# benabbouosama/DEEPL-Project

Measured on AMD Instinct MI355X. Metric: images/sec train step, TransVAE-Large f16d32 256px bs256, higher is better.
Workload: dtype bf16

## Files before the change

### deepl-project_amd/csrc/igemm_common.h

```cpp
#pragma once
#pragma clang fp contract(off)
#include "common.h"

#include <type_traits>

namespace tvi {

struct IgemmArgs {
    const bf16* x;
    const bf16* w;
    const float* bias;
    const bf16* res;
    const bf16* aux;
    bf16* pre;
    bf16* out;
    const char* zeros;
    int M, N, K;
    int batch, h_in, w_in, c_in, ldx;
    int h_out, w_out, ldo;
    int kh, kw, stride, pad, up_shift, dil_mask;
    int tiles_n, tiles_m, xcd_order;
    int sup_r, sup_c;
    int tpb, nchunks;
    int shuffle;
    int act;
    int aux_act;
    int pre_deriv;
    int form;
    const float* rope;
    int rope_tokens, rope_cols;
    int hw_shift, w_shift;
    unsigned dv_hw_m, dv_w_m, dv_cq_m;
    int dv_hw_s, dv_w_s, dv_cq_s;
    int store_nt;
    unsigned out_bytes;
    unsigned x_bytes, w_bytes;
    const bf16* x2;
    unsigned x2_bytes;
    int ldx2, k1_steps;
};

constexpr int LDS_MAX = 160 * 1024;
extern int g_cfg_bm, g_cfg_bn, g_halo_ring;
extern bool g_halo_w4, g_xcd_order, g_epi_modes;
int epilogue_mode(const IgemmArgs& a);
int pick_tile(long long M, int N, bool allow256, bool allow192_256rows, int* bm);
int launch_halo(IgemmArgs& a, hipStream_t s);
#ifdef TV_PROBE
int set_halo_probe(void* dev_buf);
#endif

}

namespace {
using namespace tvi;

#ifndef TV_NO_PIPE2
#define TV_NO_PIPE2 0
#endif
#ifndef TV_NO_LOADER_SPLIT
#define TV_NO_LOADER_SPLIT 1
#endif
#ifndef TV_HALO_VOFF_REGS
#define TV_HALO_VOFF_REGS 1
#endif
#ifndef TV_HALO_BURST
#define TV_HALO_BURST 1
#endif
#ifndef TV_GENERIC_BURST
#define TV_GENERIC_BURST 1
#endif
#ifndef TV_PIPE_ALL_MAX
// ... 672 lines not shown
```

### deepl-project_amd/csrc/igemm_nt.hip

```cpp
#include "igemm_common.h"

namespace tvi {
int g_cfg_bm = 0;
int g_cfg_bn = 0;
int g_halo_ring = 3;
bool g_halo_w4 = false;
bool g_xcd_order = true;
int g_supertile = 0;
bool g_epi_modes = true;

int epilogue_mode(const IgemmArgs& a) {
    if (a.rope) return 0;
    if (!g_epi_modes || a.shuffle || a.pre || a.out_bytes == 0) return 0;
    if (a.aux) return (a.aux_act == TV_ACT_DERIV && !a.res) ? 2 : 0;
    return (a.res && a.act == TV_ACT_NONE) ? 1 : 0;
}

int pick_tile(long long M, int N, bool allow256, bool allow192_256rows, int* bm) {
    const long long m256 = (M + 255) / 256, m128 = (M + 127) / 128;
    double best = 1e30;
    int bn = 128;
    *bm = 128;
    auto consider = [&](int cbn, int cbm, long long tiles, double slots, double eff) {
        const double rounds = (double)((long long)((tiles + slots - 1) / slots));
// ... 112 lines not shown
            } else {
                b = m / hw;
                const int r = m - b * hw;
                oy = r / p.w_out;
                ox = r - oy * p.w_out;
            }
            a_oy[it] = oy * p.stride - p.pad;
            a_ox[it] = ox * p.stride - p.pad;
            a_pix[it] = b * p.h_in * p.w_in;
        } else {
            a_oy[it] = -(1 << 28);
            a_ox[it] = 0;
            a_pix[it] = 0;
        }
    }
    const bf16* b_src[B_IT];
    bool b_ok[B_IT];
    int b_voff[B_IT];
#pragma unroll
    for (int it = 0; it < B_IT; ++it) {
        const int j = it * NW + wave;
        const int row = j * RPI + srow;
        const int rl = row % WTN;
        const int fi = bfrag_reader(rl);
        const int c = (sslot ^ swz_of<BK>(fi)) * 8;
        const int n = n0 + row;
        b_ok[it] = (j < B_INSTR) && (n < p.N);
        b_src[it] = p.w + (size_t)(b_ok[it] ? n : 0) * p.K + c;
        b_voff[it] = b_ok[it] ? (n * p.K + c) * 2 : OOB_OFFSET;
    }

    const int cch = p.c_in / BK;
#ifdef TV_ABL_K1
    const int nk = 1;
#else
    const int nk = p.kh * p.kw * cch;
#endif
    int st_ky = 0, st_kx = 0, st_ch = 0, st_t = 0;
    [[maybe_unused]] int st_i = walk_i, st_am = m0 * p.ldx * 2, st_nb = n0 * p.K * 2;
    const bf16* a_src[A_IT];
    bool a_ok[A_IT];
    int a_voff[A_IT];
    const int hv = p.h_in << p.up_shift, wv = p.w_in << p.up_shift;

    auto tap_setup = [&]() {
#pragma unroll
        for (int it = 0; it < A_IT; ++it) {
            const int uy = a_oy[it] + st_ky, ux = a_ox[it] + st_kx;
            const bool ok = ((unsigned)uy < (unsigned)hv) && ((unsigned)ux < (unsigned)wv) &&
                            (((uy | ux) & p.dil_mask) == 0);
            const int iy = uy >> p.up_shift, ix = ux >> p.up_shift;
            const int pix = a_pix[it] + iy * p.w_in + ix;
            a_ok[it] = ok;
            if constexpr (BUF) a_voff[it] = ok ? (pix * p.ldx + a_chunk[it]) * 2 : OOB_OFFSET;
            else a_src[it] = p.x + (size_t)(ok ? pix : 0) * p.ldx + a_chunk[it];
        }
    };
    tap_setup();

    bf16x8 a_reg[DMA ? 1 : A_IT], b_reg[DMA ? 1 : B_IT];

    auto issue_piece = [&](char* sbase, int q) {
        if (q < A_IT) {
            const int it = q, j = it * NW + wave;
            const int koff = st_ch * BK;
            if (A_INSTR % NW != 0 && j >= A_INSTR) {
                if constexpr (PADDED && BUF) buffer_load_lds16(p.x, p.x_bytes, smem + STAGES * STAGE, OOB_OFFSET, 0);
                else if constexpr (PADDED) __builtin_amdgcn_global_load_lds(TV_GLB(p.zeros + lane * 16), TV_LDS(smem + STAGES * STAGE), 16, 0, 0);
                return;
            }
            if constexpr (BUF) {
                buffer_load_lds16(p.x, p.x_bytes, sbase + j * 1024, a_voff[it], koff * 2 + (PERSIST ? st_am : 0));
            } else if constexpr (DMA) {
                const void* src = a_ok[it] ? (const void*)(a_src[it] + koff) : (const void*)(p.zeros + lane * 16);
                __builtin_amdgcn_global_load_lds(TV_GLB(src), TV_LDS(sbase + j * 1024), 16, 0, 0);
            } else {
// ... 7 lines not shown
            if (B_INSTR % NW != 0 && j >= B_INSTR) {
                if constexpr (PADDED && BUF) buffer_load_lds16(p.w, p.w_bytes, smem + STAGES * STAGE, OOB_OFFSET, 0);
                else if constexpr (PADDED) __builtin_amdgcn_global_load_lds(TV_GLB(p.zeros + lane * 16), TV_LDS(smem + STAGES * STAGE), 16, 0, 0);
                return;
            }
            if constexpr (BUF) {
                buffer_load_lds16(p.w, p.w_bytes, sbase + A_BYTES + j * 1024, b_voff[it], kb * 2 + (PERSIST ? st_nb : 0));
            } else if constexpr (DMA) {
                const void* src = b_ok[it] ? (const void*)(b_src[it] + kb) : (const void*)(p.zeros + lane * 16);
                __builtin_amdgcn_global_load_lds(TV_GLB(src), TV_LDS(sbase + A_BYTES + j * 1024), 16, 0, 0);
            } else {
                bf16x8 v = {0, 0, 0, 0, 0, 0, 0, 0};
                if (b_ok[it]) v = *(const bf16x8*)(b_src[it] + kb);
                b_reg[it] = v;
            }
        }
    };
    auto stage_advance = [&]() {
        if constexpr (PERSIST) {
            ++st_t;
            ++st_ch;
            if (st_t == nk) {
                st_i += p.nchunks;
                const int r = st_i / p.tiles_n, c = st_i - r * p.tiles_n;
                st_am = (r * 8 + walk_x) * (BM * p.ldx * 2);
                st_nb = c * (BN * p.K * 2);
                st_t = st_ch = 0;
            }
            return;
        }
        ++st_t;
        if (++st_ch == cch) {
            st_ch = 0;
            if (++st_kx == p.kw) {
                st_kx = 0;
                ++st_ky;
            }
            if (st_t < nk) tap_setup();
        }
    };
    auto stage_issue = [&](char* sbase) {
#pragma unroll
        for (int q = 0; q < NI; ++q) issue_piece(sbase, q);
        stage_advance();
    };
    auto stage_write = [&](char* sbase) {
        if constexpr (!DMA) {
#pragma unroll
            for (int it = 0; it < A_IT; ++it) {
                const int j = it * NW + wave;
                if (A_INSTR % NW != 0 && j >= A_INSTR) break;
                *(bf16x8*)(sbase + j * 1024 + lane * 16) = a_reg[it];
            }
#pragma unroll
            for (int it = 0; it < B_IT; ++it) {
                const int j = it * NW + wave;
                if (B_INSTR % NW != 0 && j >= B_INSTR) break;
                *(bf16x8*)(sbase + A_BYTES + j * 1024 + lane * 16) = b_reg[it];
            }
        }
    };

    int fi = lane & 15, fq = lane >> 4;
    int sw = swz_of<BK>(fi);
    int a_row_off = (wm * WTM + fi) * (BK * 2);
    int b_row_off = A_BYTES + (wn * WTN + bfrag_lane_row(fi)) * (BK * 2);
    [[maybe_unused]] auto persist_reinit = [&]() {
        int tl = threadIdx.x;
        asm volatile("" : "+v"(tl));
        const int ln = tl & 63, sr = ln / CPR, ss = ln % CPR;
#pragma unroll
// ... 466 lines not shown
            compute(smem + (t & 1) * STAGE, nullptr, std::false_type{});
            if (t + 1 < nk) stage_write(smem + ((t + 1) & 1) * STAGE);
        }
    }

    if (TV_SETPRIO) __builtin_amdgcn_s_setprio(0);
    TV_T(5);
#ifdef TV_ABL_NO_EPI
    {
        float chk = 0.f;
#pragma unroll
        for (int i = 0; i < MF; ++i)
#pragma unroll
            for (int j = 0; j < NF; ++j) chk += acc[i][j][0] + acc[i][j][1] + acc[i][j][2] + acc[i][j][3];
        if (chk != 123.456f) return;
    }
#endif
    f32x4 bvals[NF];
    load_bias<WTN>(p, lane, n0 + wn * WTN, bvals);
    const int mrow0 = m0 + wm * WTM;
    epilogue<WTM, WTN, EPI, MODE == 2 && (BM * BN >= 128 * 128)>(p, acc, bvals, smem, wave, lane, n0 + wn * WTN, [&](int r) { return mrow0 + r; });
    TV_T(6);
    TV_PROBE_DUMP(wave, lane);
}

bool g_use_dma = true;
int g_nt_threshold_mb = 64;
int g_loop8 = 1;
int g_persist = 0;
int g_cfg_stages = 0;
int g_cfg_bk = 0;
int g_addr_mode = 0;
bool g_use_halo = true;





int epilogue_form(const IgemmArgs& a) {
    if (!g_epi_modes) return EF_GENERIC;
    if (a.shuffle) {
        if (a.rope || ((a.N >> 2) % 64) != 0 || (a.N & 3)) return EF_GENERIC;
        if (a.shuffle == 1) {
            if (a.aux) return (a.aux_act == TV_ACT_DERIV && !a.res && !a.pre && a.act == TV_ACT_NONE) ? EF_DERIV_S1 : EF_GENERIC;
            if (a.pre || a.act != TV_ACT_NONE) return EF_GENERIC;
            return a.res ? EF_RES_S1 : EF_PLAIN_S1;
        }
        if (a.aux || a.res) return EF_GENERIC;
        if (a.pre) return (a.pre_deriv && a.act == TV_ACT_SILU) ? EF_SILU_D_S2 : EF_GENERIC;
        return a.act == TV_ACT_NONE ? EF_PLAIN_S2 : EF_GENERIC;
    }
    if (a.rope) return (!a.aux && !a.res && !a.pre && a.act == TV_ACT_NONE && a.rope_cols % 32 == 0) ? EF_ROPE : EF_GENERIC;
    if (a.aux) {
        if (a.aux_act == TV_ACTX_RELU) return (!a.res && !a.pre && a.act == TV_ACT_NONE) ? EF_RELU_MASK : EF_GENERIC;
        if (a.aux_act == TV_ACTX_LRELU) return (!a.res && !a.pre && a.act == TV_ACT_NONE) ? EF_LRELU_MASK : EF_GENERIC;
        if (!a.res || a.pre || a.act != TV_ACT_NONE) return EF_GENERIC;
        return a.aux_act == TV_ACT_DERIV ? EF_RES_DERIV : (a.aux_act == TV_ACT_ADD ? EF_RES2 : EF_GENERIC);
    }
    if (a.res) return EF_GENERIC;
    if (a.pre) {
        if (!a.pre_deriv) return EF_GENERIC;
        return a.act == TV_ACT_GELU ? EF_GELU_D : (a.act == TV_ACT_SILU ? EF_SILU_D : EF_GENERIC);
    }
    if (a.act == TV_ACTX_RELU) return EF_RELU;
    if (a.act == TV_ACTX_LRELU) return EF_LRELU;
    return a.act == TV_ACT_NONE ? EF_PLAIN : (a.act == TV_ACT_GELU ? EF_GELU : (a.act == TV_ACT_SILU ? EF_SILU : EF_GENERIC));
// ... 92 lines not shown
                    hipLaunchKernelGGL((igemm_nt_kernel<BM, BN, WGM, WGN, BK, STAGES, MODE, EPI_MODE, false, 0, true>), grid, block, BYTES, s, a);
                    return;
                }
            }
            hipLaunchKernelGGL((igemm_nt_kernel<BM, BN, WGM, WGN, BK, STAGES, MODE, EPI_MODE>), grid, block, BYTES, s, a);
        };
        const int epi = epilogue_mode(a);
        if constexpr (MODE == 2 && BM * BN >= 128 * 128) {
            if (epi == 1) { go(std::integral_constant<int, 1>{}); return 0; }
            if (epi == 2) { go(std::integral_constant<int, 2>{}); return 0; }
        }
        go(std::integral_constant<int, 0>{});
        return 0;
    }
}

template <int BN, int BK, int MODE>
int launch_big(const IgemmArgs& a, int bm, int stages, hipStream_t s) {
    constexpr int WGM8 = (BN == 256) ? 2 : 4, WGN8 = (BN == 256) ? 4 : 2;
    if constexpr (MODE == 0) {
        return launch_one<128, BN, 2, 2, BK, 2, 0>(a, s);
    } else {
        if (bm == 256) {
            if (stages >= 3 && launch_one<256, BN, WGM8, WGN8, BK, 3, MODE>(a, s) == 0) return 0;
            return launch_one<256, BN, WGM8, WGN8, BK, 2, MODE>(a, s);
        }
        if (stages >= 3 && launch_one<128, BN, 2, 2, BK, 3, MODE>(a, s) == 0) return 0;
        return launch_one<128, BN, 2, 2, BK, 2, MODE>(a, s);
    }
}



template <int BK, int MODE>
int launch_mode(IgemmArgs& a, hipStream_t s) {
    const int N = a.N;
    const int stages = g_cfg_stages ? g_cfg_stages : 2;
    if (N > 64) {
        int bm = 128;
        int bn = pick_tile(a.M, N, true, true, &bm);
        if (g_cfg_bn == 256 && N % 256 == 0) { bn = 256; bm = 256; }
        else if (g_cfg_bn == 192 && N % 192 == 0) { bn = 192; bm = 256; }
        else if (g_cfg_bn == 128) { bn = (N % 192 == 0 && N % 128 != 0) ? 192 : 128; bm = 128; }
        if (g_cfg_bm) bm = g_cfg_bm;
        if (bn == 256) {
            a.tiles_n = N / 256;
            return launch_big<256, BK, MODE>(a, bm, stages, s);
        }
        if (bn == 192) {
            a.tiles_n = N / 192;
            return launch_big<192, BK, MODE>(a, bm, stages, s);
        }
        a.tiles_n = (N + 127) / 128;
        return launch_big<128, BK, MODE>(a, bm, stages, s);
    }
    a.tiles_n = 1;
    if (N > 32) return launch_one<128, 64, 2, 2, BK, 2, MODE>(a, s);
    return launch_one<128, 32, 4, 1, BK, 2, MODE>(a, s);
}

template <int BK>
int launch_bk(IgemmArgs& a, hipStream_t s) {
    if (!g_use_dma) return launch_mode<BK, 0>(a, s);
    if (g_addr_mode != 1 && a.x_bytes != 0 && a.w_bytes != 0) return launch_mode<BK, 2>(a, s);
    return launch_mode<BK, 1>(a, s);
}

}

extern "C" int tv_set_dma(int on) {
    g_use_dma = on != 0;
    g_addr_mode = (on == 2) ? 1 : 0;
    return 0;
}

extern "C" int tv_set_igemm_halo(int on) {
    g_halo_w4 = on >= 100;
    on %= 100;
    g_xcd_order = on < 10;
    on %= 10;
    g_use_halo = on != 0;
    g_halo_ring = (on == 2) ? 2 : (on == 4 ? 4 : 3);
    return 0;
}

extern "C" int tv_set_igemm_nt_threshold(int mib) {
    g_nt_threshold_mb = mib;
    return 0;
}

extern "C" int tv_set_igemm_persist(int on) {
    if (on == -1) g_loop8 = 0;
    else if (on == -2) g_loop8 = 1;
    else g_persist = on;
    return 0;
}

extern "C" int tv_set_igemm_supertile(int v) {
    g_supertile = v;
    return 0;
}

extern "C" int tv_set_igemm_epilogue(int on) {
    g_epi_modes = on != 0;
    return 0;
}

#ifdef TV_PROBE
extern "C" int tv_set_igemm_probe(void* dev_buf) {
    const bool ok = hipMemcpyToSymbol(HIP_SYMBOL(g_probe_dev), &dev_buf, sizeof(void*)) == hipSuccess;
    return (tvi::set_halo_probe(dev_buf) == 0 && ok) ? 0 : 1;
}
#endif

extern "C" int tv_set_igemm_config(int bm, int bn, int stages, int bk) {
    g_cfg_bm = bm;
// ... 27 lines not shown
extern "C" int tv_igemm_nt(const tv_conv_desc* d, const void* x, const void* w, const float* bias,
                           const void* residual, void* pre_act, void* out, void* stream) {
    return igemm_nt_impl(d, x, w, bias, residual, pre_act, out, nullptr, TV_ACT_NONE, stream);
}

extern "C" int tv_igemm_nt_actgrad(const tv_conv_desc* d, const void* x, const void* w, const void* residual,
                                   const void* aux_pre_act, int aux_act, void* out, void* stream) {
    TV_CHECK_ARG(aux_pre_act && aux_act >= 0 && aux_act <= TV_ACTX_LRELU && d && d->act == TV_ACT_NONE,
                 "tv_igemm_nt_actgrad: needs the saved pre-activation, a valid activation id and desc.act == NONE");
    return igemm_nt_impl(d, x, w, nullptr, residual, nullptr, out, aux_pre_act, aux_act, stream);
}

extern "C" int tv_igemm_nt_cat2(const tv_conv_desc* d, const void* x, const void* x2, int k1, int ldx2, const void* w, const float* bias,
                               const void* residual, const void* aux, int aux_act, void* out, void* stream) {
    TV_CHECK_ARG(x2 && d && d->act == TV_ACT_NONE && (!aux || (aux_act >= 0 && aux_act <= TV_ACT_ADD && !bias)),
                 "tv_igemm_nt_cat2: needs the second source, desc.act == NONE, and no bias together with aux");
    return igemm_nt_impl(d, x, w, bias, residual, nullptr, out, aux, aux ? aux_act : TV_ACT_NONE, stream, RopeSpec{nullptr, 0, 0}, Cat2Spec{x2, k1, ldx2});
}

static int igemm_nt_impl(const tv_conv_desc* d, const void* x, const void* w, const float* bias, const void* residual,
                         void* pre_act, void* out, const void* aux, int aux_act, void* stream, RopeSpec rope, Cat2Spec cat) {
    TV_CHECK_ARG(d && x && w && out, "tv_igemm_nt: null pointer");
    if (cat.x2) {
        TV_CHECK_ARG(d->kh == 1 && d->kw == 1 && d->stride == 1 && d->pad == 0 && d->up_shift == 0 && d->dil_mask == 0 && d->store_shuffle == 0 && !rope.tab,
                     "tv_igemm_nt_cat2: single-tap layers only");
        TV_CHECK_ARG(cat.k1 > 0 && cat.k1 % 64 == 0 && d->c_in > cat.k1 && (d->c_in - cat.k1) % 64 == 0 && d->ldx >= cat.k1 && d->ldx % 8 == 0 &&
                     cat.ldx2 >= d->c_in - cat.k1 && cat.ldx2 % 8 == 0, "tv_igemm_nt_cat2: k1=%d c_in=%d ldx=%d ldx2=%d", cat.k1, d->c_in, d->ldx, cat.ldx2);
    }
    TV_CHECK_ARG(d->c_in > 0 && d->c_in % 32 == 0, "tv_igemm_nt: c_in=%d must be a multiple of 32", d->c_in);
    TV_CHECK_ARG(d->c_out > 0 && d->c_out % 8 == 0, "tv_igemm_nt: c_out=%d must be a multiple of 8", d->c_out);
    TV_CHECK_ARG(cat.x2 || (d->ldx >= d->c_in && d->ldx % 8 == 0), "tv_igemm_nt: ldx=%d (c_in=%d) must be >= c_in and a multiple of 8", d->ldx, d->c_in);
    TV_CHECK_ARG(d->ldo % 8 == 0, "tv_igemm_nt: ldo=%d must be a multiple of 8", d->ldo);
    TV_CHECK_ARG(d->batch > 0 && d->h_in > 0 && d->w_in > 0 && d->h_out > 0 && d->w_out > 0, "tv_igemm_nt: empty geometry");
    TV_CHECK_ARG(d->kh > 0 && d->kw > 0 && d->stride > 0 && d->pad >= 0, "tv_igemm_nt: bad taps");
    TV_CHECK_ARG((d->up_shift | 1) == 1 && (d->dil_mask | 1) == 1, "tv_igemm_nt: up_shift/dil_mask must be 0 or 1");
    TV_CHECK_ARG(d->act >= 0 && ((d->act & ~TV_ACT_SAVE_DERIV) <= 2 || d->act == TV_ACTX_RELU || d->act == TV_ACTX_LRELU), "tv_igemm_nt: unknown activation %d", d->act);
    TV_CHECK_ARG(!(d->act & TV_ACT_SAVE_DERIV) || (pre_act && (d->act & ~TV_ACT_SAVE_DERIV) != TV_ACT_NONE),
                 "tv_igemm_nt: TV_ACT_SAVE_DERIV needs an activation and a pre_act buffer");
    TV_CHECK_ARG((d->act != TV_ACTX_RELU && d->act != TV_ACTX_LRELU) || !pre_act, "tv_igemm_nt: a ReLU / LeakyReLU layer saves nothing (its output is its own backward mask): pre_act must be NULL");
    TV_CHECK_ARG(d->store_shuffle >= 0 && d->store_shuffle <= 2, "tv_igemm_nt: store_shuffle must be 0, 1 or 2");
    const long long M = (long long)d->batch * d->h_out * d->w_out;
    TV_CHECK_ARG(M < (1ll << 31) && (long long)d->batch * d->h_in * d->w_in < (1ll << 31), "tv_igemm_nt: too many pixels");
    if (d->store_shuffle) {
        TV_CHECK_ARG(d->c_out % 32 == 0 && d->ldo >= d->c_out / 4, "tv_igemm_nt: shuffle store needs c_out %% 32 == 0");
    } else {
        TV_CHECK_ARG(d->ldo >= d->c_out, "tv_igemm_nt: ldo < c_out");
    }
    if (tv_init() != TV_OK) return TV_ERR_INIT;

    IgemmArgs a;
    a.x = (const bf16*)x;
    a.w = (const bf16*)w;
    a.bias = bias;
    a.res = (const bf16*)residual;
    a.aux = (const bf16*)aux;
    a.aux_act = aux_act;
    a.pre = (bf16*)pre_act;
    a.out = (bf16*)out;
    a.zeros = (const char*)tv_zero_page();
    a.M = (int)M;
    a.N = d->c_out;
    a.K = d->kh * d->kw * d->c_in;
    a.batch = d->batch; a.h_in = d->h_in; a.w_in = d->w_in; a.c_in = d->c_in; a.ldx = d->ldx;
    a.h_out = d->h_out; a.w_out = d->w_out; a.ldo = d->ldo;
    a.kh = d->kh; a.kw = d->kw; a.stride = d->stride; a.pad = d->pad;
    a.up_shift = d->up_shift; a.dil_mask = d->dil_mask;
    a.tiles_n = 1;
    a.shuffle = d->store_shuffle;
    a.act = d->act & ~TV_ACT_SAVE_DERIV;
    a.pre_deriv = (d->act & TV_ACT_SAVE_DERIV) ? 1 : 0;
    a.rope = rope.tab;
    a.rope_tokens = rope.tokens;
    a.rope_cols = rope.cols;
    a.form = epilogue_form(a);
    {
        auto lg = [](int v) { int s = 0; while ((1 << s) < v) ++s; return ((1 << s) == v) ? s : -1; };
        a.w_shift = lg(d->w_out);
        a.hw_shift = lg(d->h_out * d->w_out);
        if (a.hw_shift < 0 || a.w_shift < 0) a.hw_shift = a.w_shift = -1;
    }
    {
        auto fd = [](int d, unsigned& m, int& sh) {
            if (d <= 1) { m = 0; sh = 0; return; }
            int L = 0;
            while ((1ll << L) < d) ++L;
            m = (unsigned)(((1ull << (31 + L)) + (unsigned long long)d - 1) / (unsigned long long)d);
            sh = L - 1;
        };
        fd(d->h_out * d->w_out, a.dv_hw_m, a.dv_hw_s);
        fd(d->w_out, a.dv_w_m, a.dv_w_s);
        fd(a.N >> 2, a.dv_cq_m, a.dv_cq_s);
    }
    {
        const long long rows = (long long)d->batch * d->h_in * d->w_in;
        const long long xb = (rows - 1) * d->ldx * 2 + (long long)(cat.x2 ? cat.k1 : d->c_in) * 2;
        const long long wb = (long long)a.N * a.K * 2;
        a.x_bytes = xb < (1ll << 31) ? (unsigned)xb : 0u;
        a.w_bytes = wb < (1ll << 31) ? (unsigned)wb : 0u;
        a.x2 = (const bf16*)cat.x2;
        a.ldx2 = cat.x2 ? cat.ldx2 : d->ldx;
// ... 25 lines not shown
```

### deepl-project_amd/transvae/hip/_lib.py

```python
from __future__ import annotations

import ctypes as C
import glob
import os
import subprocess
import threading

_HERE = os.path.dirname(os.path.abspath(__file__))
PKG_ROOT = os.path.dirname(os.path.dirname(_HERE))
CSRC = os.path.join(PKG_ROOT, "csrc")
SO_PATH = os.environ.get("TV_HIP_SO") or os.path.join(_HERE, "libtransvae_hip.so")

ACT_NONE, ACT_GELU, ACT_SILU = 0, 1, 2
ACT_DERIV, ACT_SAVE_DERIV = 3, 16
ACT_ADD = 4
ACTX_RELU = 5
ACTX_LRELU = 6
GAN_GEN, GAN_BCE, GAN_HINGE, GAN_WGAN = 0, 1, 2, 3
LPIPS_MAP, LPIPS_SIGMOID, LPIPS_CLAMP = 1, 2, 4
POOL3_MAX_S2, POOL3_MAX_S1P1, POOL3_AVG_S1P1 = 0, 1, 2
SSIM_SKIMAGE, SSIM_BOX11 = 0, 1
METRIC_NONE, METRIC_CLIP, METRIC_SIGMOID = 0, 1, 2
IMAGE_NONE, IMAGE_SIGMOID = 0, 1
ERR_UNSUPPORTED = 4
DERIVE_UP_FWD, DERIVE_UP_DGRAD, DERIVE_UP_WGRAD_FOLD, DERIVE_S2_PARITY = 1, 2, 3, 4


class ConvDesc(C.Structure):
    _fields_ = [(n, C.c_int) for n in (
        "batch", "h_in", "w_in", "c_in", "ldx",
        "h_out", "w_out", "c_out", "ldo",
        "kh", "kw", "stride", "pad",
        "up_shift", "dil_mask", "act", "store_shuffle")]


class ImageDesc(C.Structure):
    _fields_ = [("offset", C.c_longlong)] + [(n, C.c_int) for n in (
        "in_h", "in_w", "row_stride", "channels", "out_h", "out_w", "crop_top", "crop_left", "xtab", "xk", "ytab", "yk")]


_P, _I, _F, _LL = C.c_void_p, C.c_int, C.c_float, C.c_longlong
_DP = C.POINTER(ConvDesc)

SIGNATURES = {
    "tv_init": (_I, []),
    "tv_last_error": (C.c_char_p, []),
    "tv_abi_version": (_I, []),
    "tv_igemm_nt": (_I, [_DP, _P, _P, _P, _P, _P, _P, _P]),
    "tv_igemm_nt_rope": (_I, [_DP, _P, _P, _P, _P, _P, _I, _I, _P]),
    "tv_igemm_nt_actgrad": (_I, [_DP, _P, _P, _P, _P, _I, _P, _P]),
    "tv_igemm_nt_cat2": (_I, [_DP, _P, _P, _I, _I, _P, _P, _P, _P, _I, _P, _P]),
    "tv_wgrad_tn": (_I, [_DP, _P, _P, _P, _P, _P]),
    "tv_wgrad_tn_overwrites": (_I, [_DP]),
    "tv_wgrad_tn_acc": (_I, [_DP, _P, _P, _P, _P, _P]),
    "tv_pack_weight": (_I, [_P, _P, _P, _I, _I, _I, _I, _P]),
    "tv_conv3x3_derived": (_I, [_P, _P, _I, _I, _I, _I, _P]),
    "tv_gn_partial_count": (_LL, [_I, _I, _I]),
    "tv_gn_stats": (_I, [_P, _P, _P, _I, _I, _I, _P]),
    "tv_gn_silu_fwd": (_I, [_P, _P, _P, _P, _P, _P, _I, _I, _I, _I, _F, _P]),
    "tv_gn_silu_apply": (_I, [_P, _P, _P, _P, _P, _I, _I, _I, _I, _P]),
    "tv_gn_silu_bwd_reduce": (_I, [_P, _P, _P, _P, _P, _P, _P, _I, _I, _I, _I, _P]),
    "tv_gn_silu_bwd_apply": (_I, [_P, _P, _P, _P, _P, _P, _P, _P, _P, _P, _I, _I, _I, _I, _P]),
    "tv_rownorm_fwd": (_I, [_P, _P, _P, _I, _I, _I, _F, _F, _P]),
    "tv_rownorm_bwd": (_I, [_P, _P, _P, _P, _P, _P, _I, _I, _I, _F, _F, _P]),
    "tv_rope_qk": (_I, [_P, _P, _I, _I, _I, _I, _P]),
    "tv_attn_fwd": (_I, [_P, _P, _P, _I, _I, _I, _F, _P]),
    "tv_attn_bwd": (_I, [_P, _P, _P, _P, _P, _P, _P, _I, _I, _I, _F, _P]),
    "tv_act_bwd": (_I, [_P, _P, _P, _LL, _I, _P]),
    "tv_add_": (_I, [_P, _P, _LL, _P]),
    "tv_nchw_to_nhwc": (_I, [_P, _P, _I, _I, _I, _I, _I, _P]),
    "tv_nhwc_to_nchw": (_I, [_P, _P, _I, _I, _I, _I, _I, _P]),
    "tv_im2col3x3": (_I, [_P, _P, _I, _I, _I, _I, _I, _P]),
    "tv_pool2x2_sum": (_I, [_P, _P, _I, _I, _I, _I, _P]),
    "tv_fold_cols": (_I, [_P, _P, _P, _P, _P, _I, _I, _P]),
    "tv_fold_partial_count": (_LL, [_I, _I]),
    "tv_fold_cols_bwd": (_I, [_P, _P, _P, _P, _P, _P, _P, _P, _P, _I, _I, _P]),
    "tv_vae_loss_partial_count": (_LL, [_LL, _LL]),
    "tv_vae_loss_l1_kl": (_I, [_P, _P, _P, _P, _P, _P, _P, _P, _P, _LL, _LL, _F, _F, _F, _I, _F, _F, _P]),
    "tv_opt_chunk_elems": (_I, []),
    "tv_opt_grad_norm": (_I, [_P, _P, _I, _P, _P, _F, _F, _F, _I, _P]),
    "tv_opt_adamw": (_I, [_P, _P, _I, _P, _F, _F, _F, _F, _F, _P]),
# ... 140 lines not shown
```

### deepl-project_amd/transvae/hip/ops.py

```python
from __future__ import annotations

import contextlib
import ctypes as C
import functools
from typing import Optional

import torch

from . import _lib as L

BF16 = torch.bfloat16


def _p(t: Optional[torch.Tensor]):
    return None if t is None else C.c_void_p(t.data_ptr())


def _stream():
    return C.c_void_p(torch.cuda.current_stream().cuda_stream)


def _require(cond: bool, msg: str):
    if not cond:
        raise RuntimeError("transvae.hip: " + msg)
# ... 113 lines not shown
                        L.check(L.load().tv_pack_weight(_p(w), None, _p(dt), O, T, I, int(flip), _stream()), "tv_pack_weight")
                        ent.forms[fk] = dt
                return d, dt
    key = None
    if _pack_cache is not None and is_param:
        key = (id(base), base._version, w.data_ptr(), O, T, I, want_fwd, want_t, flip)
        hit = _pack_cache.get(key)
        if hit is not None:
            return hit
    d = torch.empty((O, T, I), dtype=BF16, device=w.device) if want_fwd else None
    dt = torch.empty((I, T, O), dtype=BF16, device=w.device) if want_t else None
    lib = L.load()
    L.check(lib.tv_pack_weight(_p(w), _p(d), _p(dt), O, T, I, int(flip), _stream()), "tv_pack_weight")
    if key is not None:
        _pack_cache[key] = (d, dt)
    return d, dt


def _derived_weight(w: torch.Tensor, kind: str, build):
    if _pack_cache is None:
        return build()
    base = w._base if w._base is not None else w
    if not isinstance(base, torch.nn.Parameter):
        return build()
    key = (id(base), base._version, w.data_ptr(), tuple(w.shape), kind)
    hit = _pack_cache.get(key)
    if hit is None:
        hit = _pack_cache[key] = build()
    return hit


def _desc(**kw) -> L.ConvDesc:
    d = L.ConvDesc()
    for k in ("up_shift", "dil_mask", "act", "store_shuffle", "pad"):
        setattr(d, k, 0)
    d.stride = 1
    for k, v in kw.items():
        setattr(d, k, int(v))
    return d


_LAUNCH_BYTES = (1 << 31) - (1 << 26)


def _batch_chunks(batch: int, tensors, align: int = 1):
    per_row = 0
    for t in tensors:
        if t is not None:
            per_row = max(per_row, (t.numel() // batch) * t.element_size())
    if per_row * batch < _LAUNCH_BYTES:
        return None
    rows = max(align, (_LAUNCH_BYTES // per_row) // align * align)
    n = -(-batch // rows)
    rows = -(-(-(-batch // n)) // align) * align
    return [(s, min(rows, batch - s)) for s in range(0, batch, rows)]


def _row_ptr(t, batch: int, row: int):
    if t is None:
        return None
    return C.c_void_p(t.data_ptr() + row * (t.numel() // batch) * t.element_size())


def _desc_rows(desc: L.ConvDesc, rows: int) -> L.ConvDesc:
    d = L.ConvDesc()
    C.memmove(C.byref(d), C.byref(desc), C.sizeof(L.ConvDesc))
    d.batch = rows
# ... 245 lines not shown
        lib = L.load()
        B = desc.batch
        for s, c in (_batch_chunks(B, (gz, residual, aux, dx)) or [(0, B)]):
            L.check(lib.tv_igemm_nt_actgrad(C.byref(_desc_rows(desc, c)), _row_ptr(gz, B, s), _p(wt), _row_ptr(residual, B, s),
                                            _row_ptr(aux, B, s), aux_act, _row_ptr(dx, B, s), _stream()), "tv_igemm_nt_actgrad")


_UP_SETS = (((0,), (1, 2)), ((0, 1), (2,)))


def _derive(w: torch.Tensor, form: int, Cout: int, Cin: int, out: torch.Tensor, accumulate: bool = False) -> torch.Tensor:
    _require(w.dtype == torch.float32 and w.is_contiguous() and out.is_contiguous(), "derived operand needs contiguous fp32 input")
    L.check(L.load().tv_conv3x3_derived(_p(w), _p(out), form, Cout, Cin, int(accumulate), _stream()), "tv_conv3x3_derived")
    return out


def _up_fwd_weight(w: torch.Tensor, Cout: int, Cin: int) -> torch.Tensor:
    return _derive(w.view(Cout, 3, 3, Cin), L.DERIVE_UP_FWD, Cout, Cin, torch.empty((4 * Cout, 2, 2, Cin), dtype=BF16, device=w.device))


_UP_ADJ = ((2,), (1, 2), (0, 1), (0,))


def _up_dgrad_weight(w: torch.Tensor, Cout: int, Cin: int) -> torch.Tensor:
    return _derive(w.view(Cout, 3, 3, Cin), L.DERIVE_UP_DGRAD, Cout, Cin, torch.empty((Cin, 4, 4, Cout), dtype=BF16, device=w.device))


def _up_fold_wgrad(d16: torch.Tensor, Cout: int, Cin: int, out: Optional[torch.Tensor] = None, accumulate: bool = False) -> torch.Tensor:
    if out is None:
        out = torch.empty((Cout, 3, 3, Cin), dtype=torch.float32, device=d16.device)
    return _derive(d16, L.DERIVE_UP_WGRAD_FOLD, Cout, Cin, out, accumulate)


def _s2_parity_weight(w: torch.Tensor, Cout: int, Cin: int) -> torch.Tensor:
    return _derive(w.view(Cout, 3, 3, Cin), L.DERIVE_S2_PARITY, Cout, Cin, torch.empty((4 * Cin, 2, 2, Cout), dtype=BF16, device=w.device))


def _rows_desc(rows: int, c_in: int, c_out: int) -> L.ConvDesc:
    return _desc(batch=rows, h_in=1, w_in=1, c_in=c_in, ldx=c_in, h_out=1, w_out=1, c_out=c_out, ldo=c_out, kh=1, kw=1)


def gemm_rows(x: torch.Tensor, wb: torch.Tensor, c_out: int, bias=None, residual=None, aux=None, aux_act: int = 0) -> torch.Tensor:
    T, K = x.shape
    out = torch.empty((T, c_out), dtype=BF16, device=x.device)
    d = _rows_desc(T, K, c_out)
    if aux is None:
        igemm(d, x, wb, bias, residual, None, out)
    else:
        _require(bias is None, "gemm_rows: bias and a derivative multiply do not combine")
        _igemm_bwd(d, x, wb, residual, aux, aux_act, out)
    return out


def gemm_rows2(x1: torch.Tensor, x2: torch.Tensor, wb: torch.Tensor, c_out: int, bias=None, residual=None, aux=None, aux_act: int = 0):
    T, K1 = x1.shape
    K2 = x2.shape[1]
    _require(x1.dtype == BF16 and x2.dtype == BF16 and x1.is_contiguous() and x2.is_contiguous() and x2.shape[0] == T and
             wb.dtype == BF16 and wb.is_contiguous() and
             (tuple(wb.shape[-2:]) == (c_out, K1 + K2) or wb.numel() == c_out * (K1 + K2)), "gemm_rows2: operand check failed")
    if K1 % 64 or K2 % 64 or _batch_chunks(T, (x1, x2, residual, aux)) is not None:
        return None
    d = _rows_desc(T, K1 + K2, c_out)
    d.ldx = K1
    out = torch.empty((T, c_out), dtype=BF16, device=x1.device)
    rc = L.load().tv_igemm_nt_cat2(C.byref(d), _p(x1), _p(x2), K1, K2, _p(wb), _p(bias), _p(residual), _p(aux), int(aux_act), _p(out), _stream())
    if rc == 4:
# ... 129 lines not shown


def _c4s2_poly_weight(w: torch.Tensor, Cout: int, Cin: int) -> torch.Tensor:
    wt = w.permute(3, 1, 2, 0)
    out = torch.empty((4, Cin, 2, 2, Cout), dtype=BF16, device=w.device)
    for py in range(2):
        for px in range(2):
            sel = wt[:, list(_C4S2_KY[py])][:, :, list(_C4S2_KY[px])]
            out[2 * py + px] = sel.to(BF16)
    return out.view(4 * Cin, 2, 2, Cout)


def conv_dgrad(g: _Geo, w, gz, x_shape, residual=None, aux=None, aux_act: int = 0):
    lib = L.load()
    m = g.mode
    T = g.KH * g.KW
    dev = gz.device
    if m == "unshuf":
        _, wt = pack_weight(w.view(g.Cout, 1, T * g.Cin), False, True, False)
    elif m in ("c3s2", "c3up") or (m == "c4s2" and C4S2_DGRAD_FORM == "polyphase"):
        wt = None
    else:
        _, wt = pack_weight(w.view(g.Cout, T, g.Cin), False, True, m in ("c3s1", "c4s1", "c4s2"))
    dx = torch.empty(x_shape, dtype=BF16, device=dev)
    if m == "linear":
        d = _desc(batch=g.B, h_in=1, w_in=1, c_in=g.Cout, ldx=g.Cout, h_out=1, w_out=1, c_out=g.Cin, ldo=g.Cin, kh=1, kw=1)
        _igemm_bwd(d, gz, wt, residual, aux, aux_act, dx)
    elif m == "c3s1":
        d = _desc(batch=g.B, h_in=g.H, w_in=g.W, c_in=g.Cout, ldx=g.Cout, h_out=g.H, w_out=g.W, c_out=g.Cin, ldo=g.Cin,
                  kh=3, kw=3, stride=1, pad=1)
        _igemm_bwd(d, gz, wt, residual, aux, aux_act, dx)
    elif m == "c3s2":
        wd = _derived_weight(w, "s2_parity", lambda: _s2_parity_weight(w, g.Cout, g.Cin))
        d = _desc(batch=g.B, h_in=g.Ho, w_in=g.Wo, c_in=g.Cout, ldx=g.Cout, h_out=g.Ho, w_out=g.Wo, c_out=4 * g.Cin, ldo=g.Cin,
                  kh=2, kw=2, stride=1, pad=0, store_shuffle=1)
        _igemm_bwd(d, gz, wd, residual, aux, aux_act, dx)
    elif m == "c3up":
        wd = _derived_weight(w, "up_dgrad", lambda: _up_dgrad_weight(w, g.Cout, g.Cin))
        d = _desc(batch=g.B, h_in=g.Ho, w_in=g.Wo, c_in=g.Cout, ldx=g.Cout, h_out=g.H, w_out=g.W, c_out=g.Cin, ldo=g.Cin,
                  kh=4, kw=4, stride=2, pad=1)
        _igemm_bwd(d, gz, wd, residual, aux, aux_act, dx)
    elif m == "c4s1":
        d = _desc(batch=g.B, h_in=g.Ho, w_in=g.Wo, c_in=g.Cout, ldx=g.Cout, h_out=g.H, w_out=g.W, c_out=g.Cin, ldo=g.Cin,
                  kh=4, kw=4, stride=1, pad=2)
        _igemm_bwd(d, gz, wt, residual, aux, aux_act, dx)
    elif m == "c4s2" and C4S2_DGRAD_FORM == "polyphase":
        wd = _derived_weight(w, "c4s2_poly", lambda: _c4s2_poly_weight(w, g.Cout, g.Cin))
        d = _desc(batch=g.B, h_in=g.Ho, w_in=g.Wo, c_in=g.Cout, ldx=g.Cout, h_out=g.Ho + 1, w_out=g.Wo + 1, c_out=4 * g.Cin,
                  ldo=g.Cin, kh=2, kw=2, stride=1, pad=1, store_shuffle=2)
        _igemm_bwd(d, gz, wd, residual, aux, aux_act, dx)
    elif m == "c4s2":
        d = _desc(batch=g.B, h_in=g.Ho, w_in=g.Wo, c_in=g.Cout, ldx=g.Cout, h_out=g.H, w_out=g.W, c_out=g.Cin, ldo=g.Cin,
                  kh=4, kw=4, stride=1, pad=2, up_shift=1, dil_mask=1)
        _igemm_bwd(d, gz, wt, residual, aux, aux_act, dx)
    elif m == "unshuf":
        d = _desc(batch=g.B, h_in=g.Ho, w_in=g.Wo, c_in=g.Cout, ldx=g.Cout, h_out=g.Ho, w_out=g.Wo, c_out=4 * g.Cin, ldo=g.Cin,
                  kh=1, kw=1, store_shuffle=1)
        _igemm_bwd(d, gz, wt, residual, aux, aux_act, dx)
    elif m == "shuf":
        cq = g.Cout // 4
        d = _desc(batch=g.B, h_in=2 * g.H, w_in=2 * g.W, c_in=cq, ldx=cq, h_out=g.H, w_out=g.W, c_out=g.Cin, ldo=g.Cin,
                  kh=2, kw=2, stride=2, pad=0)
        _igemm_bwd(d, gz, wt, residual, aux, aux_act, dx)
    else:
        raise ValueError(m)
    return dx


def _wgrad_overwrites(desc: L.ConvDesc) -> bool:
# ... 307 lines not shown
```

### include/transvae_hip.h

```cpp
#ifndef TRANSVAE_HIP_H
#define TRANSVAE_HIP_H

#include <stdint.h>

#ifdef __cplusplus
extern "C" {
#endif

#define TV_OK 0
#define TV_ERR_ARG 1
#define TV_ERR_LAUNCH 2
#define TV_ERR_INIT 3
#define TV_ERR_UNSUPPORTED 4

#define TV_ACT_NONE 0
#define TV_ACT_GELU 1
#define TV_ACT_SILU 2
#define TV_ACT_DERIV 3
#define TV_ACT_ADD 4
#define TV_ACT_SAVE_DERIV 16
#define TV_ACTX_RELU 5
#define TV_ACTX_LRELU 6

int tv_init(void);
const char* tv_last_error(void);
int tv_abi_version(void);

typedef struct tv_conv_desc {
    int batch, h_in, w_in, c_in, ldx;
    int h_out, w_out, c_out, ldo;
    int kh, kw, stride, pad;
    int up_shift, dil_mask;
    int act;
    int store_shuffle;
} tv_conv_desc;

int tv_igemm_nt(const tv_conv_desc* d, const void* x, const void* w, const float* bias,
                const void* residual, void* pre_act, void* out, void* stream);

int tv_igemm_nt_rope(const tv_conv_desc* d, const void* x, const void* w, const float* bias, void* out,
                     const float* rope_tab, int tokens_per_image, int rope_cols, void* stream);

int tv_igemm_nt_actgrad(const tv_conv_desc* d, const void* x, const void* w, const void* residual,
                        const void* aux_pre_act, int aux_act, void* out, void* stream);

int tv_igemm_nt_cat2(const tv_conv_desc* d, const void* x, const void* x2, int k1, int ldx2, const void* w, const float* bias,
                     const void* residual, const void* aux, int aux_act, void* out, void* stream);

int tv_wgrad_tn(const tv_conv_desc* d, const void* x, const void* gy, float* dw, float* dbias,
                void* stream);
int tv_wgrad_tn_overwrites(const tv_conv_desc* d);
int tv_wgrad_tn_acc(const tv_conv_desc* d, const void* x, const void* gy, float* dw, float* dbias, void* stream);

int tv_pack_weight(const float* src, void* dst, void* dst_t, int O, int T, int I, int flip_taps,
                   void* stream);

#define TV_DERIVE_UP_FWD 1
#define TV_DERIVE_UP_DGRAD 2
#define TV_DERIVE_UP_WGRAD_FOLD 3
#define TV_DERIVE_S2_PARITY 4
int tv_conv3x3_derived(const float* src, void* dst, int form, int c_out, int c_in, int accumulate, void* stream);

long long tv_gn_partial_count(int batch, int hw, int C);
int tv_gn_stats(const void* x, float* stats, float* partials, int batch, int hw, int C, void* stream);
int tv_gn_silu_fwd(const void* x, const float* stats, const float* gamma, const float* beta,
                   float* mr, void* y, int batch, int hw, int C, int G, float eps, void* stream);
int tv_gn_silu_apply(const void* x, const float* mr, const float* gamma, const float* beta, void* y,
                     int batch, int hw, int C, int G, void* stream);
int tv_gn_silu_bwd_reduce(const void* x, const void* dy, const float* mr, const float* gamma,
                          const float* beta, float* red, float* partials, int batch, int hw, int C,
                          int G, void* stream);
// ... 170 lines not shown
```

Measured before the change: 161.6.

## Skip structurally zero taps per quadrant in stride-2 parity dgrad igemm

Adds a per-quadrant tap mask to the implicit-GEMM conv so that each N-tile loops only over the live taps of its output-parity quadrant. The stride-2 3x3 dgrad expressed as a 2x2 parity conv is the only caller, and it has known all-zero taps in three of four quadrants. Tile selection is adjusted so that N tiles align to quadrant boundaries when K is large. This removes wasted MFMA and load work on zero weights, at the cost of uneven work across N tiles and extra loop logic for advancing between taps.

```diff
diff --git a/deepl-project_amd/csrc/igemm_common.h b/deepl-project_amd/csrc/igemm_common.h
--- a/deepl-project_amd/csrc/igemm_common.h
+++ b/deepl-project_amd/csrc/igemm_common.h
@@ -38,6 +38,7 @@
     const bf16* x2;
     unsigned x2_bytes;
     int ldx2, k1_steps;
+    unsigned tap_mask;
 };
 
 constexpr int LDS_MAX = 160 * 1024;
diff --git a/deepl-project_amd/csrc/igemm_nt.hip b/deepl-project_amd/csrc/igemm_nt.hip
--- a/deepl-project_amd/csrc/igemm_nt.hip
+++ b/deepl-project_amd/csrc/igemm_nt.hip
@@ -168,16 +168,33 @@
 
     const int cch = p.c_in / BK;
 #ifdef TV_ABL_K1
-    const int nk = 1;
+    unsigned st_live = 1u;
 #else
-    const int nk = p.kh * p.kw * cch;
-#endif
+    unsigned st_live = (1u << (p.kh * p.kw)) - 1u;
+    if (p.tap_mask) {
+        const int nq = p.N >> 2;
+        const int q = (n0 >= nq) + (n0 >= 2 * nq) + (n0 >= 3 * nq);
+        st_live = (p.tap_mask >> (4 * q)) & 15u;
+    }
+#endif
+    const int nk = __builtin_popcount(st_live) * cch;
     int st_ky = 0, st_kx = 0, st_ch = 0, st_t = 0;
     [[maybe_unused]] int st_i = walk_i, st_am = m0 * p.ldx * 2, st_nb = n0 * p.K * 2;
     const bf16* a_src[A_IT];
     bool a_ok[A_IT];
     int a_voff[A_IT];
     const int hv = p.h_in << p.up_shift, wv = p.w_in << p.up_shift;
+    [[maybe_unused]] auto tap_next = [&]() {
+        for (;;) {
+            st_live >>= 1;
+            if (++st_kx == p.kw) {
+                st_kx = 0;
+                ++st_ky;
+            }
+            if (!st_live || (st_live & 1u)) break;
+            st_t += cch;
+        }
+    };
 
     auto tap_setup = [&]() {
 #pragma unroll
@@ -251,11 +268,8 @@
         ++st_t;
         if (++st_ch == cch) {
             st_ch = 0;
-            if (++st_kx == p.kw) {
-                st_kx = 0;
-                ++st_ky;
-            }
-            if (st_t < nk) tap_setup();
+            tap_next();
+            if (st_live) tap_setup();
         }
     };
     auto stage_issue = [&](char* sbase) {
@@ -788,6 +802,7 @@
 int g_cfg_bk = 0;
 int g_addr_mode = 0;
 bool g_use_halo = true;
+bool g_tapskip = true;
 
 
 
@@ -946,17 +961,36 @@
 
 
 
+constexpr int TAPSKIP_RETILE_MIN_K = 1536;
+int choose_tile(long long M, int N, int K, unsigned tap_mask, int* bm) {
+    *bm = 128;
+    if (N <= 32) return 32;
+    if (N <= 64) return 64;
+    int bn = pick_tile(M, N, true, true, bm);
+    if (tap_mask && g_tapskip && K >= TAPSKIP_RETILE_MIN_K && !(N & 3) && (N >> 2) % bn != 0) {
+        if ((N >> 2) % 192 == 0) { bn = 192; *bm = 256; }
+        else if ((N >> 2) % 128 == 0) { bn = 128; *bm = 128; }
+    }
+    if (g_cfg_bn == 256 && N % 256 == 0) { bn = 256; *bm = 256; }
+    else if (g_cfg_bn == 192 && N % 192 == 0) { bn = 192; *bm = 256; }
+    else if (g_cfg_bn == 128) { bn = (N % 192 == 0 && N % 128 != 0) ? 192 : 128; *bm = 128; }
+    if (g_cfg_bm) *bm = g_cfg_bm;
+    return bn;
+}
+
+unsigned usable_tap_mask(unsigned mask, int N, int bn) {
+    if (!g_tapskip || !mask || (N & 3) || (N >> 2) % bn != 0) return 0u;
+    return mask;
+}
+
 template <int BK, int MODE>
 int launch_mode(IgemmArgs& a, hipStream_t s) {
     const int N = a.N;
     const int stages = g_cfg_stages ? g_cfg_stages : 2;
+    int bm = 128;
+    const int bn = choose_tile(a.M, N, a.K, a.tap_mask, &bm);
+    a.tap_mask = usable_tap_mask(a.tap_mask, N, bn);
     if (N > 64) {
-        int bm = 128;
-        int bn = pick_tile(a.M, N, true, true, &bm);
-        if (g_cfg_bn == 256 && N % 256 == 0) { bn = 256; bm = 256; }
-        else if (g_cfg_bn == 192 && N % 192 == 0) { bn = 192; bm = 256; }
-        else if (g_cfg_bn == 128) { bn = (N % 192 == 0 && N % 128 != 0) ? 192 : 128; bm = 128; }
-        if (g_cfg_bm) bm = g_cfg_bm;
         if (bn == 256) {
             a.tiles_n = N / 256;
             return launch_big<256, BK, MODE>(a, bm, stages, s);
@@ -996,6 +1030,37 @@
     g_use_halo = on != 0;
     g_halo_ring = (on == 2) ? 2 : (on == 4 ? 4 : 3);
     return 0;
+}
+
+extern "C" int tv_set_igemm_tapskip(int on) {
+    const int was = g_tapskip ? 1 : 0;
+    g_tapskip = on != 0;
+    return was;
+}
+
+static const char* tap_mask_error(const tv_conv_desc* d) {
+    if (!d->tap_mask) return nullptr;
+    const int taps = d->kh * d->kw;
+    if ((unsigned)d->tap_mask > 0xffffu || taps > 4 || (d->c_out & 3)) return "tap_mask needs at most 4 taps and c_out % 4 == 0";
+    for (int q = 0; q < 4; ++q) {
+        const unsigned m = ((unsigned)d->tap_mask >> (4 * q)) & 15u;
+        if (!(m & 1u) || (m >> taps)) return "tap_mask: tap 0 must be live in every quadrant, and no bit beyond kh*kw may be set";
+    }
+    return nullptr;
+}
+
+extern "C" int tv_igemm_tapskip_plan(const tv_conv_desc* d) {
+    if (!d || d->batch <= 0 || d->h_out <= 0 || d->w_out <= 0 || d->c_out <= 0 || d->kh <= 0 || d->kw <= 0) {
+        tv_set_error("tv_igemm_tapskip_plan: bad descriptor");
+        return -1;
+    }
+    if (const char* err = tap_mask_error(d)) {
+        tv_set_error("tv_igemm_tapskip_plan: %s", err);
+        return -1;
+    }
+    int bm;
+    const int bn = choose_tile((long long)d->batch * d->h_out * d->w_out, d->c_out, d->kh * d->kw * d->c_in, (unsigned)d->tap_mask, &bm);
+    return usable_tap_mask((unsigned)d->tap_mask, d->c_out, bn) ? 1 : 0;
 }
 
 extern "C" int tv_set_igemm_nt_threshold(int mib) {
@@ -1089,7 +1154,11 @@
     TV_CHECK_ARG(cat.x2 || (d->ldx >= d->c_in && d->ldx % 8 == 0), "tv_igemm_nt: ldx=%d (c_in=%d) must be >= c_in and a multiple of 8", d->ldx, d->c_in);
     TV_CHECK_ARG(d->ldo % 8 == 0, "tv_igemm_nt: ldo=%d must be a multiple of 8", d->ldo);
     TV_CHECK_ARG(d->batch > 0 && d->h_in > 0 && d->w_in > 0 && d->h_out > 0 && d->w_out > 0, "tv_igemm_nt: empty geometry");
-    TV_CHECK_ARG(d->kh > 0 && d->kw > 0 && d->stride > 0 && d->pad >= 0, "tv_igemm_nt: bad taps");
+    TV_CHECK_ARG(d->kh > 0 && d->kw > 0 && d->kh * d->kw <= 31 && d->stride > 0 && d->pad >= 0, "tv_igemm_nt: bad taps");
+    {
+        const char* err = tap_mask_error(d);
+        TV_CHECK_ARG(!err, "tv_igemm_nt: %s", err ? err : "");
+    }
     TV_CHECK_ARG((d->up_shift | 1) == 1 && (d->dil_mask | 1) == 1, "tv_igemm_nt: up_shift/dil_mask must be 0 or 1");
     TV_CHECK_ARG(d->act >= 0 && ((d->act & ~TV_ACT_SAVE_DERIV) <= 2 || d->act == TV_ACTX_RELU || d->act == TV_ACTX_LRELU), "tv_igemm_nt: unknown activation %d", d->act);
     TV_CHECK_ARG(!(d->act & TV_ACT_SAVE_DERIV) || (pre_act && (d->act & ~TV_ACT_SAVE_DERIV) != TV_ACT_NONE),
@@ -1123,6 +1192,7 @@
     a.kh = d->kh; a.kw = d->kw; a.stride = d->stride; a.pad = d->pad;
     a.up_shift = d->up_shift; a.dil_mask = d->dil_mask;
     a.tiles_n = 1;
+    a.tap_mask = (unsigned)d->tap_mask;
     a.shuffle = d->store_shuffle;
     a.act = d->act & ~TV_ACT_SAVE_DERIV;
     a.pre_deriv = (d->act & TV_ACT_SAVE_DERIV) ? 1 : 0;
diff --git a/deepl-project_amd/transvae/hip/_lib.py b/deepl-project_amd/transvae/hip/_lib.py
--- a/deepl-project_amd/transvae/hip/_lib.py
+++ b/deepl-project_amd/transvae/hip/_lib.py
@@ -31,7 +31,7 @@
         "batch", "h_in", "w_in", "c_in", "ldx",
         "h_out", "w_out", "c_out", "ldo",
         "kh", "kw", "stride", "pad",
-        "up_shift", "dil_mask", "act", "store_shuffle")]
+        "up_shift", "dil_mask", "act", "store_shuffle", "tap_mask")]
 
 
 class ImageDesc(C.Structure):
@@ -47,6 +47,8 @@
     "tv_last_error": (C.c_char_p, []),
     "tv_abi_version": (_I, []),
     "tv_igemm_nt": (_I, [_DP, _P, _P, _P, _P, _P, _P, _P]),
+    "tv_igemm_tapskip_plan": (_I, [_DP]),
+    "tv_set_igemm_tapskip": (_I, [_I]),
     "tv_igemm_nt_rope": (_I, [_DP, _P, _P, _P, _P, _P, _I, _I, _P]),
     "tv_igemm_nt_actgrad": (_I, [_DP, _P, _P, _P, _P, _I, _P, _P]),
     "tv_igemm_nt_cat2": (_I, [_DP, _P, _P, _I, _I, _P, _P, _P, _P, _I, _P, _P]),
diff --git a/deepl-project_amd/transvae/hip/ops.py b/deepl-project_amd/transvae/hip/ops.py
--- a/deepl-project_amd/transvae/hip/ops.py
+++ b/deepl-project_amd/transvae/hip/ops.py
@@ -169,7 +169,7 @@
 
 def _desc(**kw) -> L.ConvDesc:
     d = L.ConvDesc()
-    for k in ("up_shift", "dil_mask", "act", "store_shuffle", "pad"):
+    for k in ("up_shift", "dil_mask", "act", "store_shuffle", "pad", "tap_mask"):
         setattr(d, k, 0)
     d.stride = 1
     for k, v in kw.items():
@@ -481,6 +481,14 @@
     return _derive(d16, L.DERIVE_UP_WGRAD_FOLD, Cout, Cin, out, accumulate)
 
 
+S2_PARITY_TAP_MASK = 0xF531
+
+
+def _s2_parity_desc(g) -> L.ConvDesc:
+    return _desc(batch=g.B, h_in=g.Ho, w_in=g.Wo, c_in=g.Cout, ldx=g.Cout, h_out=g.Ho, w_out=g.Wo, c_out=4 * g.Cin, ldo=g.Cin,
+                 kh=2, kw=2, stride=1, pad=0, store_shuffle=1, tap_mask=S2_PARITY_TAP_MASK)
+
+
 def _s2_parity_weight(w: torch.Tensor, Cout: int, Cin: int) -> torch.Tensor:
     return _derive(w.view(Cout, 3, 3, Cin), L.DERIVE_S2_PARITY, Cout, Cin, torch.empty((4 * Cin, 2, 2, Cout), dtype=BF16, device=w.device))
 
@@ -676,9 +684,7 @@
         _igemm_bwd(d, gz, wt, residual, aux, aux_act, dx)
     elif m == "c3s2":
         wd = _derived_weight(w, "s2_parity", lambda: _s2_parity_weight(w, g.Cout, g.Cin))
-        d = _desc(batch=g.B, h_in=g.Ho, w_in=g.Wo, c_in=g.Cout, ldx=g.Cout, h_out=g.Ho, w_out=g.Wo, c_out=4 * g.Cin, ldo=g.Cin,
-                  kh=2, kw=2, stride=1, pad=0, store_shuffle=1)
-        _igemm_bwd(d, gz, wd, residual, aux, aux_act, dx)
+        _igemm_bwd(_s2_parity_desc(g), gz, wd, residual, aux, aux_act, dx)
     elif m == "c3up":
         wd = _derived_weight(w, "up_dgrad", lambda: _up_dgrad_weight(w, g.Cout, g.Cin))
         d = _desc(batch=g.B, h_in=g.Ho, w_in=g.Wo, c_in=g.Cout, ldx=g.Cout, h_out=g.H, w_out=g.W, c_out=g.Cin, ldo=g.Cin,
diff --git a/include/transvae_hip.h b/include/transvae_hip.h
--- a/include/transvae_hip.h
+++ b/include/transvae_hip.h
@@ -33,10 +33,14 @@
     int up_shift, dil_mask;
     int act;
     int store_shuffle;
+    int tap_mask;
 } tv_conv_desc;
 
 int tv_igemm_nt(const tv_conv_desc* d, const void* x, const void* w, const float* bias,
                 const void* residual, void* pre_act, void* out, void* stream);
+
+int tv_igemm_tapskip_plan(const tv_conv_desc* d);
+int tv_set_igemm_tapskip(int on);
 
 int tv_igemm_nt_rope(const tv_conv_desc* d, const void* x, const void* w, const float* bias, void* out,
                      const float* rope_tab, int tokens_per_image, int rope_cols, void* stream);
```

Result: no change. 161.4 (-0.1%).
